# Onr/Council-GAN

Hardware: NVIDIA H100
Metric: training images/sec (gen+dis step) (higher is better)
Workload: dtype tf32

## Files before the change

council_gan_b200/csrc/api.cu:

```cuda
#include "common.cuh"
#include <string.h>

namespace cg {

static thread_local char g_err[512] = "";
std::atomic<uint64_t> g_launches{0};
thread_local int g_tc_mode = 7;
thread_local int g_pdl = 0;

void set_error(const char* fmt, ...) {
    va_list ap;
    va_start(ap, fmt);
    vsnprintf(g_err, sizeof(g_err), fmt, ap);
    va_end(ap);
}

int validate_geom(const cg_conv_geom& g) {
    CG_REQUIRE(g.G >= 1 && (g.x_groups == 1 || g.x_groups == g.G), "conv: x_groups=%d must be 1 or G=%d", g.x_groups, g.G);
    CG_REQUIRE(g.Cin % 4 == 0 && g.Cin > 0, "conv: Cin=%d must be a positive multiple of 4", g.Cin);
    CG_REQUIRE(g.Cout > 0 && g.B > 0 && g.H > 0 && g.W > 0, "conv: empty tensor");
    CG_REQUIRE(g.stride >= 1 && g.KH >= 1 && g.KW >= 1 && g.pad >= 0, "conv: bad kernel geometry");
    int Hin = g.ups ? 2 * g.H : g.H, Win = g.ups ? 2 * g.W : g.W;
    int Ho = (Hin + 2 * g.pad - g.KH) / g.stride + 1, Wo = (Win + 2 * g.pad - g.KW) / g.stride + 1;
    CG_REQUIRE(Ho == g.Ho && Wo == g.Wo, "conv: output size %dx%d inconsistent with geometry (expected %dx%d)", g.Ho, g.Wo, Ho, Wo);
// ... 83 lines not shown
        set_error("cudaGetDevice: %s", cudaGetErrorString(e));
        return CG_ERR_NO_DEVICE;
    }
    cudaDeviceProp prop;
    e = cudaGetDeviceProperties(&prop, dev);
    if (e != cudaSuccess) {
        set_error("cudaGetDeviceProperties: %s", cudaGetErrorString(e));
        return CG_ERR_NO_DEVICE;
    }
    if (sm_count) *sm_count = prop.multiProcessorCount;
    if (cc_major) *cc_major = prop.major;
    if (cc_minor) *cc_minor = prop.minor;
    return prop.multiProcessorCount;
}

extern "C" int cg_set_tensor_core_mode(int mode) {
    int prev = g_tc_mode;
    g_tc_mode = mode == 1 ? 7 : (mode & 7);
    g_small_bn = ((mode >> 23) & 1) ? 0 : 1;
    g_wgrad_tma = ((mode >> 25) & 1) ? 0 : 1;
    g_pdl = (mode >> 22) & 1;
    g_tc_serial_epilogue = (mode >> 26) & 1;
    g_tc_reg_epilogue = (mode >> 27) & 1;
    return prev;
}

extern "C" uint64_t cg_launch_count(void) { return g_launches.load(); }
extern "C" void cg_tensor_map_cache_stats(uint64_t* hits, uint64_t* misses) { tc_map_cache_stats(hits, misses); }

extern "C" int cg_zero(void* ptr, size_t bytes, void* stream) {
    cudaError_t e = cudaMemsetAsync(ptr, 0, bytes, (cudaStream_t)stream);
    if (e != cudaSuccess) {
        set_error("cg_zero: %s", cudaGetErrorString(e));
        return CG_ERR_CUDA;
    }
    return CG_OK;
}

extern "C" size_t cg_conv_workspace_bytes(const cg_conv_geom* g, int which) {
    if (!g) return 0;
    ConvDims d = conv_dims(*g);
    size_t need = 0;
    const bool patch_fwd = which == 0 && (g_tc_mode & 1) && patch_path(*g) && g->KH * g->KW >= 16;
    if (which == 2 && small_wgrad_supported(*g)) return small_ws(*g, 2);
    if (which == 1 && small_dgrad_supported(*g)) return small_ws(*g, 1);
    const bool patch_wgrad = which == 2 && (g_tc_mode & 4) && patch_path(*g);
// ... 138 lines not shown
```

council_gan_b200/csrc/common.cuh:

```cuda
#pragma once
#include <cuda.h>
#include <cuda_runtime.h>
#include <stdint.h>
#include <stdio.h>
#include <stdarg.h>
#include <atomic>
#include "../../include/council_b200.h"

namespace cg {

void set_error(const char* fmt, ...);
extern std::atomic<uint64_t> g_launches;
extern thread_local int g_tc_mode;
extern thread_local int g_small_bn;
extern thread_local int g_wgrad_tma;
extern thread_local int g_tc_serial_epilogue;
extern thread_local int g_tc_reg_epilogue;

constexpr int CG_MAX_DEVICES = 64;
inline int current_device() {
    int dev = 0;
    cudaGetDevice(&dev);
    return dev >= 0 && dev < CG_MAX_DEVICES ? dev : 0;
}
struct PerDeviceOnce {
    std::atomic<bool> done[CG_MAX_DEVICES];
    bool first() { return !done[current_device()].exchange(true); }
    void reset() { done[current_device()].store(false); }
};

inline int check_launch(const char* what) {
    g_launches.fetch_add(1, std::memory_order_relaxed);
    cudaError_t e = cudaGetLastError();
    if (e != cudaSuccess) {
        set_error("%s: %s", what, cudaGetErrorString(e));
        return CG_ERR_CUDA;
    }
    return CG_OK;
}

// ... 93 lines not shown
```

council_gan_b200/csrc/conv_tc.cu:

```cuda
#include "common.cuh"
#include "tc_ptx.cuh"
#include <cstdlib>
#include <cstdio>
#include <cuda.h>
#include <mutex>
#include <string.h>

namespace cg {

typedef CUresult (*EncodeTiledFn)(CUtensorMap*, CUtensorMapDataType, cuuint32_t, void*, const cuuint64_t*, const cuuint64_t*,
                                  const cuuint32_t*, const cuuint32_t*, CUtensorMapInterleave, CUtensorMapSwizzle,
                                  CUtensorMapL2promotion, CUtensorMapFloatOOBfill);
typedef CUresult (*EncodeIm2colFn)(CUtensorMap*, CUtensorMapDataType, cuuint32_t, void*, const cuuint64_t*, const cuuint64_t*,
                                   const int*, const int*, cuuint32_t, cuuint32_t, const cuuint32_t*, CUtensorMapInterleave,
                                   CUtensorMapSwizzle, CUtensorMapL2promotion, CUtensorMapFloatOOBfill);
typedef CUresult (*ReplaceAddressFn)(CUtensorMap*, void*);
static EncodeTiledFn g_encode_tiled = nullptr;
static ReplaceAddressFn g_replace_address = nullptr;
static EncodeIm2colFn g_encode_im2col = nullptr;
static int g_sm_count_dev[CG_MAX_DEVICES] = {0};
static int sm_count_now() {
    int dev = current_device();
    if (!g_sm_count_dev[dev]) cudaDeviceGetAttribute(&g_sm_count_dev[dev], cudaDevAttrMultiProcessorCount, dev);
    return g_sm_count_dev[dev];
}
thread_local int g_small_bn = 1;
thread_local int g_tc_serial_epilogue = 0;
thread_local int g_tc_reg_epilogue = 0;
static int g_driver_version = 0;
static std::once_flag g_once;

struct MapKey {
    const void* ptr;
    int64_t a, b;
    int32_t v[8];
    bool operator==(const MapKey& o) const { return ptr == o.ptr && a == o.a && b == o.b && memcmp(v, o.v, sizeof(v)) == 0; }
};
struct MapSlot {
    MapKey key;
    CUtensorMap map;
    bool used;
};
constexpr int MAP_SLOTS = 8192;
static MapSlot* g_map_cache = nullptr;
static std::mutex g_map_mutex;
static std::atomic<uint64_t> g_map_hits{0}, g_map_misses{0};
static inline uint32_t map_hash(const MapKey& k) {
    uint64_t h = 1469598103934665603ull;
    const unsigned char* p = reinterpret_cast<const unsigned char*>(&k);
    for (size_t i = 0; i < sizeof(MapKey); i++) h = (h ^ p[i]) * 1099511628211ull;
    return (uint32_t)(h ^ (h >> 32)) & (MAP_SLOTS - 1);
// ... 57 lines not shown
struct TcParams {
    CUtensorMap bmap;
    TcClass cls[TC_MAX_CLASSES];
    int ncls;
    int G, xg_images;
    int B, P, Q;
    int Cin, Cout, KH, KW, stride;
    int bn;
    int bk;
    int cps;
    int n_store;
    int out_H, out_W, out_sh, out_sw;
    int w_rows_per_group;
    float* y; const float* bias; const float* addend; const float* mask_src;
    float* stats;
    long stats_gbc;
    int act; float slope;
    int stages;
    int serial_epilogue;
    CUtensorMap ymap, addmap, maskmap;
    int epi_slots, epi_slot_bytes;
};

__device__ __forceinline__ void tc_tile(const TcParams& p, int t, int MT, int NT, int& mt, int& nt, int& c, int& g) {
    if (p.serial_epilogue) {
        mt = t % MT;
        int r = t / MT;
        nt = r % NT;
        r /= NT;
        c = r % p.ncls;
        g = r / p.ncls;
        return;
    }
    c = t % p.ncls;
    int r = t / p.ncls;
    mt = r % MT;
    r /= MT;
    nt = r % NT;
    g = r / NT;
}

__device__ __forceinline__ void tc_half_coords(const TcParams& p, int g, int mt, int h, int& q, int& n) {
    const int pq = p.P * p.Q;
    const int m = mt * TC_BM + 64 * h;
    const int img = m / pq, rem = m - img * pq;
    const int pp = rem / p.Q;
    q = rem - pp * p.Q;
    n = (g * p.B + img) * (p.out_H / p.out_sh) + pp;
}

template <int BK, int BN>
__global__ void __launch_bounds__(TC_THREADS, 1) conv_tc_kernel(const __grid_constant__ TcParams p) {
    pdl_trigger();
    extern __shared__ __align__(1024) uint8_t smem_raw[];
    uint8_t* smem = reinterpret_cast<uint8_t*>((reinterpret_cast<uintptr_t>(smem_raw) + 1023) & ~(uintptr_t)1023);
    const int wg = __shfl_sync(0xffffffffu, threadIdx.x >> 7, 0), tid = threadIdx.x & 127;
    constexpr int a_bytes = TC_BM * BK * 4;
    constexpr int b_bytes = ((BN * BK * 4) + 1023) & ~1023;
    const int stage_bytes = p.cps * (a_bytes + b_bytes);
    constexpr int tx_chunk = a_bytes + BN * BK * 4;
    constexpr bool tma_epi = BK == 32 && BN >= 64;
    const int epi_slots = tma_epi ? p.epi_slots : 0;
    uint8_t* epi = smem + (size_t)p.stages * stage_bytes;
    uint64_t* full_bar = reinterpret_cast<uint64_t*>(epi + (size_t)epi_slots * p.epi_slot_bytes);
    uint64_t* empty_bar = full_bar + p.stages;
    uint64_t* efull_bar = empty_bar + p.stages;
    uint64_t* eempty_bar = efull_bar + epi_slots;

    const int MT = (p.B * p.P * p.Q + TC_BM - 1) / TC_BM;
    const int NT = (p.Cout + BN - 1) / BN;
    const int tiles = p.G * p.ncls * NT * MT;
    const int kchunks = (p.Cin + BK - 1) / BK;
    const int kiters = p.KH * p.KW * kchunks;

    if (threadIdx.x == 0) {
        prefetch_tmap(&p.bmap);
        for (int c = 0; c < p.ncls; c++) prefetch_tmap(&p.cls[c].amap);
        for (int s = 0; s < p.stages; s++) {
            mbar_init(&full_bar[s], 1);
            mbar_init(&empty_bar[s], 2);
        }
        if (epi_slots) {
            prefetch_tmap(&p.ymap);
            if (p.addend) prefetch_tmap(&p.addmap);
            if (p.mask_src) prefetch_tmap(&p.maskmap);
        }
        for (int s = 0; s < epi_slots; s++) {
            mbar_init(&efull_bar[s], 1);
            mbar_init(&eempty_bar[s], 2);
        }
        fence_barrier_init();
    }
    __syncthreads();
    pdl_wait();

    if (wg == 0) {
        if (tid == 0) {
            int stage = 0;
            uint32_t phase = 0;
            for (int t = blockIdx.x; t < tiles; t += gridDim.x) {
                int mt, nt, c, g;
                tc_tile(p, t, MT, NT, mt, nt, c, g);
                const TcClass& cl = p.cls[c];
                long m0 = (long)mt * TC_BM;
                int img = (int)(m0 / (p.P * p.Q));
                int rem = (int)(m0 - (long)img * p.P * p.Q);
                int pp = rem / p.Q, qq = rem - pp * p.Q;
                int n_coord = g * p.xg_images + img;
                int w_coord = cl.w0 + qq * p.stride;
                int h_coord = cl.h0 + pp * p.stride;
                int wrow = g * p.w_rows_per_group + cl.wrow_off + nt * BN;
                int kh = 0, kw = 0, kc = 0;
                for (int k0 = 0; k0 < kiters; k0 += p.cps) {
                    const int n = kiters - k0 < p.cps ? kiters - k0 : p.cps;
                    mbar_wait(&empty_bar[stage], phase ^ 1);
                    uint8_t* sa = smem + (size_t)stage * stage_bytes;
                    uint8_t* sb = sa + p.cps * a_bytes;
                    mbar_expect_tx(&full_bar[stage], (uint32_t)(n * tx_chunk));
                    for (int j = 0; j < n; j++) {
                        tma_load_im2col_4d(&cl.amap, &full_bar[stage], sa + j * a_bytes, kc * BK, w_coord, h_coord, n_coord, (uint16_t)kw,
                                           (uint16_t)kh);
                        tma_load_2d(&p.bmap, &full_bar[stage], sb + j * b_bytes, (kh * p.KW + kw) * p.Cin + kc * BK, wrow);
                        if (++kc == kchunks) { kc = 0; if (++kw == p.KW) { kw = 0; ++kh; } }
                    }
                    if (++stage == p.stages) { stage = 0; phase ^= 1; }
                }
            }
        } else if (tid == 32 && epi_slots) {
            const uint32_t ebytes = (p.addend ? 2 * 8192 : 0) + (p.mask_src ? 2 * 8192 : 0);
            int es = 0;
            uint32_t ephase = 0;
            for (int t = blockIdx.x; t < tiles; t += gridDim.x) {
                int mt, nt, c, g;
                tc_tile(p, t, MT, NT, mt, nt, c, g);
                const TcClass& cl = p.cls[c];
                int q[2], n[2];
                tc_half_coords(p, g, mt, 0, q[0], n[0]);
                tc_half_coords(p, g, mt, 1, q[1], n[1]);
                for (int sl = 0; sl < BN / 32; sl++) {
                    mbar_wait(&eempty_bar[es], ephase ^ 1);
                    if (ebytes) {
                        mbar_expect_tx(&efull_bar[es], ebytes);
                        uint8_t* dst = epi + (size_t)es * p.epi_slot_bytes;
                        const int c0 = nt * BN + 32 * sl;
                        for (int h = 0; h < 2; h++) {
                            if (p.addend) tma_load_5d(&p.addmap, &efull_bar[es], dst + h * 8192, c0, cl.out_w0, q[h], cl.out_h0, n[h]);
                            if (p.mask_src)
                                tma_load_5d(&p.maskmap, &efull_bar[es], dst + (p.addend ? 16384 : 0) + h * 8192, c0, cl.out_w0, q[h],
                                            cl.out_h0, n[h]);
                        }
                    } else {
                        mbar_arrive(&efull_bar[es]);
                    }
                    if (++es == epi_slots) { es = 0; ephase ^= 1; }
                }
            }
        }
        return;
    }

    const int cw = wg - 1;
    const int warp4 = tid >> 5, lane = tid & 31;
    const int row0 = cw * 64 + warp4 * 16 + (lane >> 2);
    const int cq = 2 * (lane & 3);
    const uint64_t desc0 = BK == 32 ? make_kmajor_sw128_desc(0) : make_kmajor_sw32_desc(0);
    float acc[BN / 2];
    int stage = 0;
    uint32_t phase = 0;
    int es = 0;
    uint32_t ephase = 0;
    for (int t = blockIdx.x; t < tiles; t += gridDim.x) {
        int mt, nt, c, g;
        tc_tile(p, t, MT, NT, mt, nt, c, g);
        const TcClass& cl = p.cls[c];
        int prev = -1;
        for (int k0 = 0; k0 < kiters; k0 += p.cps) {
            const int n = kiters - k0 < p.cps ? kiters - k0 : p.cps;
            mbar_wait(&full_bar[stage], phase);
            const uint32_t sa = smem_u32(smem + (size_t)stage * stage_bytes) + cw * (64 * BK * 4);
            const uint32_t sb = smem_u32(smem + (size_t)stage * stage_bytes) + p.cps * a_bytes;
            wgmma_fence();
            for (int j = 0; j < n; j++) {
                const uint64_t adesc = desc0 | (uint64_t)(((sa + j * a_bytes) & 0x3FFFF) >> 4);
                const uint64_t bdesc = desc0 | (uint64_t)(((sb + j * b_bytes) & 0x3FFFF) >> 4);
#pragma unroll
                for (int kk = 0; kk < BK / 8; kk++)
                    wgmma_tf32<BN>(acc, adesc + (uint64_t)(kk * 2), bdesc + (uint64_t)(kk * 2), (k0 | j | kk) != 0 ? 1 : 0);
            }
            wgmma_commit();
            wgmma_wait<1>();
            if (prev >= 0 && tid == 0) mbar_arrive(&empty_bar[prev]);
            prev = stage;
            if (++stage == p.stages) { stage = 0; phase ^= 1; }
        }
        wgmma_wait<0>();
        wgmma_reg_fence(acc, BN / 2);
        if (tid == 0) mbar_arrive(&empty_bar[prev]);

        const int pq = p.P * p.Q;
        long out_off[2];
        bool valid[2];
#pragma unroll
        for (int h = 0; h < 2; h++) {
            const int m = mt * TC_BM + row0 + 8 * h;
            valid[h] = m < p.B * pq;
            out_off[h] = 0;
            if (valid[h]) {
                int img = m / pq;
                int rem = m - img * pq;
                int pp = rem / p.Q, qq = rem - pp * p.Q;
                long pix = ((long)(g * p.B + img) * p.out_H + (pp * p.out_sh + cl.out_h0)) * p.out_W + (qq * p.out_sw + cl.out_w0);
                out_off[h] = pix * p.Cout + nt * p.n_store;
            }
        }
        if (p.stats) {
            const int tiles_per_img = pq / TC_BM;
            const int img = (mt * TC_BM) / pq;
            const int chunk = ((c * tiles_per_img + (mt - img * tiles_per_img)) << 3) + cw * 4 + warp4;
            const bool b2 = lane & 4, b3 = lane & 8;
            float* st = p.stats + ((long)chunk * p.stats_gbc + (long)(g * p.B + img) * p.Cout + nt * BN + cq) * 2 + (b3 ? 2 : 0) + (b2 ? 1 : 0);
#pragma unroll
            for (int j = 0; j < BN / 8; j++) {
                const float s0 = acc[4 * j] + acc[4 * j + 2], s1 = acc[4 * j + 1] + acc[4 * j + 3];
                const float q0 = acc[4 * j] * acc[4 * j] + acc[4 * j + 2] * acc[4 * j + 2];
                const float q1 = acc[4 * j + 1] * acc[4 * j + 1] + acc[4 * j + 3] * acc[4 * j + 3];
                const float k0 = b2 ? q0 : s0, k1 = b2 ? q1 : s1;
                const float r0 = __shfl_xor_sync(0xffffffffu, b2 ? s0 : q0, 4), r1 = __shfl_xor_sync(0xffffffffu, b2 ? s1 : q1, 4);
                const float x0 = k0 + r0, x1 = k1 + r1;
                float v = (b3 ? x1 : x0) + __shfl_xor_sync(0xffffffffu, b3 ? x0 : x1, 8);
                v += __shfl_xor_sync(0xffffffffu, v, 16);
                if (lane < 16) st[16 * j] = v;
            }
        }
        if constexpr (tma_epi) {
            if (epi_slots) {
                int q, n;
                tc_half_coords(p, g, mt, cw, q, n);
                const int r0 = warp4 * 16 + (lane >> 2);
#pragma unroll
                for (int sl = 0; sl < BN / 32; sl++) {
                    float2 bv[4];
#pragma unroll
                    for (int jj = 0; jj < 4; jj++)
                        bv[jj] = p.bias ? __ldg(reinterpret_cast<const float2*>(p.bias + (long)g * p.Cout + nt * BN + 32 * sl + 8 * jj + cq))
                                        : make_float2(0.f, 0.f);
                    mbar_wait(&efull_bar[es], ephase);
                    uint8_t* half = epi + (size_t)es * p.epi_slot_bytes + cw * 8192;
                    const uint8_t* msk = half + (p.addend ? 16384 : 0);
#pragma unroll
                    for (int jj = 0; jj < 4; jj++) {
                        const int j = 4 * sl + jj;
#pragma unroll
                        for (int h = 0; h < 2; h++) {
                            const int r = r0 + 8 * h;
                            const int off = r * 128 + (((2 * jj + (cq >> 2)) ^ (r & 7)) << 4) + (cq & 3) * 4;
                            float2 o = make_float2(acc[4 * j + 2 * h] + bv[jj].x, acc[4 * j + 2 * h + 1] + bv[jj].y);
                            if (p.addend) {
                                const float2 a = *reinterpret_cast<const float2*>(half + off);
                                o.x += a.x; o.y += a.y;
                            }
                            if (p.mask_src) {
                                const float2 a = *reinterpret_cast<const float2*>(msk + off);
                                o.x *= a.x > 0.f ? 1.f : p.slope; o.y *= a.y > 0.f ? 1.f : p.slope;
                            } else if (p.act != CG_ACT_NONE) {
                                o.x = apply_act(o.x, p.act, p.slope); o.y = apply_act(o.y, p.act, p.slope);
                            }
                            *reinterpret_cast<float2*>(half + off) = o;
                        }
                    }
                    fence_proxy_async();
                    named_bar_sync(1 + cw, 128);
                    if (tid == 0) {
                        tma_store_5d(&p.ymap, half, nt * BN + 32 * sl, cl.out_w0, q, cl.out_h0, n);
                        bulk_commit();
                        if (sl > 0) {
                            bulk_wait_read<1>();
                            mbar_arrive(&eempty_bar[es == 0 ? epi_slots - 1 : es - 1]);
                        }
                        if (sl == BN / 32 - 1) {
                            bulk_wait_read<0>();
                            mbar_arrive(&eempty_bar[es]);
                        }
                    }
                    if (++es == epi_slots) { es = 0; ephase ^= 1; }
                }
                continue;
            }
        }
        if (!(p.addend || p.mask_src) || p.serial_epilogue) {
#pragma unroll
            for (int j = 0; j < BN / 8; j++) {
                const int col = 8 * j + cq;
// ... 52 lines not shown


static int encode_weights_map_raw(CUtensorMap* map, const float* w, long rows, long ktot, int bn, int bk) {
    cuuint64_t dims[2] = {(cuuint64_t)ktot, (cuuint64_t)rows};
    cuuint64_t strides[1] = {(cuuint64_t)ktot * 4};
    cuuint32_t box[2] = {(cuuint32_t)bk, (cuuint32_t)bn};
    cuuint32_t estr[2] = {1, 1};
    CUresult r = g_encode_tiled(map, CU_TENSOR_MAP_DATA_TYPE_TFLOAT32, 2, (void*)w, dims, strides, box, estr,
                                CU_TENSOR_MAP_INTERLEAVE_NONE, bk == 32 ? CU_TENSOR_MAP_SWIZZLE_128B : CU_TENSOR_MAP_SWIZZLE_32B,
                                CU_TENSOR_MAP_L2_PROMOTION_L2_256B, CU_TENSOR_MAP_FLOAT_OOB_FILL_NONE);
    if (r != CUDA_SUCCESS) {
        set_error("cuTensorMapEncodeTiled(weights rows=%ld ktot=%ld bn=%d) failed: %d", rows, ktot, bn, (int)r);
        return CG_ERR_CUDA;
    }
    return CG_OK;
}

static int encode_weights_map(CUtensorMap* map, const float* w, long rows, long ktot, int bn, int bk = TC_BK) {
    MapKey k{};
    k.ptr = w; k.a = rows; k.b = ktot; k.v[0] = bn; k.v[1] = bk; k.v[7] = 1;
    return cached_map(map, k, [&](CUtensorMap* m) { return encode_weights_map_raw(m, w, rows, ktot, bn, bk); });
}

static int encode_weights_map_p(TcParams& p, const float* w, long rows, long ktot) {
    return encode_weights_map(&p.bmap, w, rows, ktot, p.bn, p.bk);
}

static int encode_act_map_raw(CUtensorMap* map, const float* x, long N, int H, int W, int C, int lo_w, int lo_h, int up_w, int up_h,
                              int stride, int bk) {
    cuuint64_t dims[4] = {(cuuint64_t)C, (cuuint64_t)W, (cuuint64_t)H, (cuuint64_t)N};
    cuuint64_t strides[3] = {(cuuint64_t)C * 4, (cuuint64_t)W * C * 4, (cuuint64_t)H * W * C * 4};
    int lower[2] = {lo_w, lo_h};
    int upper[2] = {up_w, up_h};
    cuuint32_t estr[4] = {1, (cuuint32_t)stride, (cuuint32_t)stride, 1};
    CUresult r = g_encode_im2col(map, CU_TENSOR_MAP_DATA_TYPE_TFLOAT32, 4, (void*)x, dims, strides, lower, upper, bk, TC_BM, estr,
                                 CU_TENSOR_MAP_INTERLEAVE_NONE, bk == 32 ? CU_TENSOR_MAP_SWIZZLE_128B : CU_TENSOR_MAP_SWIZZLE_32B,
                                 CU_TENSOR_MAP_L2_PROMOTION_L2_128B, CU_TENSOR_MAP_FLOAT_OOB_FILL_NONE);
    if (r != CUDA_SUCCESS) {
        set_error("cuTensorMapEncodeIm2col(N=%ld H=%d W=%d C=%d corners %d,%d / %d,%d stride %d) failed: %d", N, H, W, C, lo_w, lo_h,
                  up_w, up_h, stride, (int)r);
        return CG_ERR_CUDA;
    }
    if (g_driver_version <= 13010 && (long)N * H * W * C * 4 < 131072) reinterpret_cast<uint64_t*>(map)[1] &= ~(1ull << 21);
    return CG_OK;
}

static int encode_act_map(CUtensorMap* map, const float* x, long N, int H, int W, int C, int lo_w, int lo_h, int up_w, int up_h,
                          int stride, int bk = TC_BK) {
    MapKey k{};
    k.ptr = x; k.a = N; k.b = ((int64_t)H << 32) | (uint32_t)W;
// ... 49 lines not shown

bool tc_fwd_supported(const cg_conv_geom& g) {
    init_driver();
    if (!g_encode_tiled || !g_encode_im2col) return false;
    if (g.ups && !(g.KH == 3 && g.KW == 3 && g.stride == 1 && g.pad == 1 && g.Cin % TC_BK == 0)) return false;
    if (pick_bk(g.Cin) == 0) return false;
    if (pick_bn(g.Cout) == 0) return false;
    if (g.pad > 120 || g.KH > 120) return false;
    if ((long)g.B * (g.ups ? g.H * g.W : g.Ho * g.Wo) < TC_BM) return false;
    return true;
}

template <int BK>
static void (*tc_kernel_for(int bn))(TcParams) {
    switch (bn) {
        case 16: return conv_tc_kernel<BK, 16>;
        case 64: return conv_tc_kernel<BK, 64>;
        case 128: return conv_tc_kernel<BK, 128>;
        case 256: return conv_tc_kernel<BK, 256>;
    }
    return nullptr;
}

static int launch_tc(TcParams& p, cudaStream_t st) {
    int a_bytes = TC_BM * p.bk * 4, b_bytes = ((p.bn * p.bk * 4) + 1023) & ~1023;
    int chunk_bytes = a_bytes + b_bytes;
    int kiters = p.KH * p.KW * ((p.Cin + p.bk - 1) / p.bk);
    int cps = p.bn <= 64 ? 2 : 1;
    if (p.bk == 8) cps = 8;
    while (cps > 1 && (cps > kiters || cps * chunk_bytes > 64 * 1024)) cps >>= 1;
    p.cps = cps;
    int stage_bytes = cps * chunk_bytes;
    int stages = (226 * 1024 - 1024 - 2 * TC_MAX_STAGES * 8) / stage_bytes;
    if (stages > TC_MAX_STAGES) stages = TC_MAX_STAGES;
    if (stages > 4 && stage_bytes >= 48 * 1024) stages = 4;
    if (p.n_store == 0) p.n_store = p.bn;
    p.serial_epilogue = g_tc_serial_epilogue;
    p.epi_slots = 0;
    const int nops = (p.addend ? 1 : 0) + (p.mask_src ? 1 : 0);
    const bool aligned = ((uintptr_t)p.y | (uintptr_t)p.addend | (uintptr_t)p.mask_src) % 16 == 0;
    if (g_replace_address && !g_tc_reg_epilogue && !p.serial_epilogue && p.bk == TC_BK && p.bn >= 64 && p.n_store == p.bn && (long)p.P * p.Q % TC_BM == 0 &&
        (p.Q % 64 == 0 || 64 % p.Q == 0) && p.out_H % p.out_sh == 0 && p.out_W % p.out_sw == 0 && p.Cout % 4 == 0 && aligned) {
        const int slot_bytes = (nops ? nops : 1) * 16384;
        auto slots_beside = [&](int st) { return (int)((227L * 1024 - 1024 - (long)st * stage_bytes - 2 * st * 8) / (slot_bytes + 16)); };
        while (slots_beside(stages) < 2 && stages > 4) stages--;
        const int e = slots_beside(stages);
        if (e >= 2) {
            p.epi_slots = e < 4 ? e : 4;
            p.epi_slot_bytes = slot_bytes;
            const long ni = (long)p.G * p.B;
            const int qbox = p.Q < 64 ? p.Q : 64;
            if (int rc = encode_out_map(&p.ymap, p.y, ni, p.out_H, p.out_W, p.Cout, p.out_sh, p.out_sw, qbox)) return rc;
            if (p.addend)
                if (int rc = encode_out_map(&p.addmap, p.addend, ni, p.out_H, p.out_W, p.Cout, p.out_sh, p.out_sw, qbox)) return rc;
            if (p.mask_src)
                if (int rc = encode_out_map(&p.maskmap, p.mask_src, ni, p.out_H, p.out_W, p.Cout, p.out_sh, p.out_sw, qbox)) return rc;
        }
    }
    p.stages = stages;
    size_t smem = (size_t)stages * stage_bytes + 1024  + 2 * stages * 8 + (size_t)p.epi_slots * (p.epi_slot_bytes + 16);
    void (*kern)(TcParams) = p.bk == 32 ? tc_kernel_for<32>(p.bn) : tc_kernel_for<8>(p.bn);
    if (!kern) {
        set_error("conv_tc: no kernel for N tile %d / K chunk %d", p.bn, p.bk);
        return CG_ERR_ARG;
    }
    static PerDeviceOnce attr_set;
    if (attr_set.first()) {
        for (int bn : {16, 64, 128, 256}) {
            cudaError_t e = cudaFuncSetAttribute(tc_kernel_for<32>(bn), cudaFuncAttributeMaxDynamicSharedMemorySize, 227 * 1024);
            if (e == cudaSuccess) e = cudaFuncSetAttribute(tc_kernel_for<8>(bn), cudaFuncAttributeMaxDynamicSharedMemorySize, 227 * 1024);
            if (e != cudaSuccess) {
                attr_set.reset();
                set_error("cudaFuncSetAttribute(conv_tc_kernel): %s", cudaGetErrorString(e));
                return CG_ERR_CUDA;
            }
        }
    }
    int MT = cdiv((long)p.B * p.P * p.Q, TC_BM);
    long tiles = (long)p.G * p.ncls * ((p.Cout + p.bn - 1) / p.bn) * MT;
    const long slots = sm_count_now();
    int grid = (int)(tiles < slots ? tiles : slots);
    launch_k(kern, grid, TC_THREADS, smem, st, p);
    return check_launch("conv_tc_kernel");
}


__global__ void ups_weight_transform_kernel(const float* __restrict__ w, float* __restrict__ wc, long total, int Cout, int Cin) {
    pdl_trigger();
    pdl_wait();
    long i = (long)blockIdx.x * blockDim.x + threadIdx.x;
    if (i >= total) return;
    int ci = (int)(i % Cin);
    long t = i / Cin;
    int ss = (int)(t % 2); t /= 2;
    int r = (int)(t % 2); t /= 2;
    int co = (int)(t % Cout); t /= Cout;
    int cls = (int)(t % 4);
    int g = (int)(t / 4);
// ... 22 lines not shown
                size_t ws_bytes, cudaStream_t st, float* stats_part) {
    init_driver();
    TcParams p{};
    p.stats = stats_part;
    p.stats_gbc = (long)g.G * g.B * g.Cout;
    p.bn = pick_bn(g.Cout);
    if (p.bn > 64) p.bn = fill_bn(p.bn, (long)g.B * (g.ups ? g.H * g.W : g.Ho * g.Wo), g.G * (g.ups ? 4 : 1), g.Cout);
    p.n_store = p.bn == 16 ? g.Cout : p.bn;
    p.bk = pick_bk(g.Cin);
    long nimg = (long)(g.x_groups == 1 ? 1 : g.G) * g.B;
    p.G = g.G; p.xg_images = g.x_groups == 1 ? 0 : g.B;
    p.B = g.B; p.Cin = g.Cin; p.Cout = g.Cout;
    p.y = y; p.bias = bias; p.addend = nullptr; p.mask_src = nullptr; p.act = act; p.slope = slope;
    if (g.ups) {
        size_t need = tc_fwd_ws(g);
        if (need > ws_bytes) {
            set_error("conv_fwd(tc, upsample classes): workspace %zu < %zu bytes", ws_bytes, need);
            return CG_ERR_WORKSPACE;
        }
        float* wc = (float*)ws;
        long total = (long)g.G * 4 * g.Cout * 4 * g.Cin;
        launch_k(ups_weight_transform_kernel, cdiv(total, 256), 256, 0, st, w, wc, total, g.Cout, g.Cin);
        if (int rc = check_launch("ups_weight_transform")) return rc;
        if (int rc = encode_weights_map_p(p, wc, (long)g.G * 4 * g.Cout, 4L * g.Cin)) return rc;
        for (int c = 0; c < 4; c++) {
            int a = c >> 1, b = c & 1;
            int lo_h = a == 0 ? -1 : 0, lo_w = b == 0 ? -1 : 0;
            int up_h = a == 0 ? -1 : 0, up_w = b == 0 ? -1 : 0;
            if (int rc = encode_act_map(&p.cls[c].amap, x, nimg, g.H, g.W, g.Cin, lo_w, lo_h, up_w, up_h, 1, p.bk)) return rc;
            p.cls[c].w0 = lo_w; p.cls[c].h0 = lo_h; p.cls[c].out_h0 = a; p.cls[c].out_w0 = b; p.cls[c].wrow_off = c * g.Cout;
        }
        p.ncls = 4;
        p.P = g.H; p.Q = g.W; p.KH = 2; p.KW = 2; p.stride = 1;
        p.out_H = g.Ho; p.out_W = g.Wo; p.out_sh = 2; p.out_sw = 2;
        p.w_rows_per_group = 4 * g.Cout;
        return launch_tc(p, st);
    }
    long ktot = (long)g.KH * g.KW * g.Cin;
    if (int rc = encode_weights_map_p(p, w, (long)g.G * g.Cout, ktot)) return rc;
    if (int rc = encode_act_map(&p.cls[0].amap, x, nimg, g.H, g.W, g.Cin, -g.pad, -g.pad, g.pad - (g.KW - 1), g.pad - (g.KH - 1), g.stride,
                                p.bk))
        return rc;
    p.cls[0].w0 = -g.pad; p.cls[0].h0 = -g.pad; p.cls[0].out_h0 = 0; p.cls[0].out_w0 = 0; p.cls[0].wrow_off = 0;
    p.ncls = 1;
    p.P = g.Ho; p.Q = g.Wo;
    p.KH = g.KH; p.KW = g.KW; p.stride = g.stride;
    p.out_H = g.Ho; p.out_W = g.Wo; p.out_sh = 1; p.out_sw = 1;
    p.w_rows_per_group = g.Cout;
    return launch_tc(p, st);
}

__global__ void __launch_bounds__(256) dgrad_weight_transform_kernel(const float* __restrict__ w, float* __restrict__ wt, int Cout, int Cin,
                                                                     int CinP, int KH, int KW, int s) {
    pdl_trigger();
    pdl_wait();
    __shared__ float tile[32][33];
    const int TH = KH / s, TW = KW / s;
    const int cit = (CinP + 31) / 32;
    const int co0 = (blockIdx.x / cit) * 32, ci0 = (blockIdx.x % cit) * 32;
    int t = blockIdx.y;
    const int ss = t % TW; t /= TW;
    const int r = t % TH; t /= TH;
    const int cls = t;
    const int g = blockIdx.z;
    const int ph = cls / s, pw = cls - ph * s;
    const int kh = ph + s * (TH - 1 - r), kw = pw + s * (TW - 1 - ss);
    const int tx = threadIdx.x, ty = threadIdx.y;
#pragma unroll
    for (int j = 0; j < 4; j++) {
        const int co = co0 + ty + 8 * j, ci = ci0 + tx;
        tile[ty + 8 * j][tx] = (co < Cout && ci < Cin) ? __ldg(w + ((((long)g * Cout + co) * KH + kh) * KW + kw) * Cin + ci) : 0.f;
    }
// ... 30 lines not shown
    init_driver();
    size_t need = tc_dgrad_ws(g);
    if (need > ws_bytes) {
        set_error("conv_dgrad(tc): workspace %zu < %zu bytes", ws_bytes, need);
        return CG_ERR_WORKSPACE;
    }
    const int s = g.stride, TH = g.KH / s, TW = g.KW / s, ncls = s * s;
    const int Hin = g.ups ? 2 * g.H : g.H, Win = g.ups ? 2 * g.W : g.W;
    float* wt = (float*)ws;
    const int CinP = g.Cin <= 16 ? 16 : g.Cin;
    size_t wt_bytes = ((size_t)g.G * g.Cout * g.KH * g.KW * CinP * sizeof(float) + 1023) & ~(size_t)1023;
    float* d_seen = g.ups ? (float*)((uint8_t*)ws + wt_bytes) : dx;
    long total = (long)g.G * g.Cout * g.KH * g.KW * CinP;
    (void)total;
    launch_k(dgrad_weight_transform_kernel, dim3(cdiv(g.Cout, 32) * cdiv(CinP, 32), g.KH * g.KW, g.G), dim3(32, 8), 0, st, w, wt, g.Cout, g.Cin, CinP,
                                                                                                                  g.KH, g.KW, s);
    if (int rc = check_launch("dgrad_weight_transform")) return rc;

    TcParams p{};
    p.bn = pick_bn(g.Cin);
    if (p.bn > 64) p.bn = fill_bn(p.bn, (long)g.B * ((g.ups ? 2 * g.H : g.H) / g.stride) * ((g.ups ? 2 * g.W : g.W) / g.stride), g.G * g.stride * g.stride, g.Cin);
    p.n_store = p.bn == 16 ? g.Cin : p.bn;
    p.bk = pick_bk(g.Cout);
    long ktot = (long)TH * TW * g.Cout;
    if (int rc = encode_weights_map_p(p, wt, (long)g.G * ncls * CinP, ktot)) return rc;
    for (int c = 0; c < ncls; c++) {
        int ph = c / s, pw = c - ph * s;
        int ihf = ((ph - g.pad) % s + s) % s, iwf = ((pw - g.pad) % s + s) % s;
        int padl_h = (TH - 1) - (ihf + g.pad - ph) / s, padl_w = (TW - 1) - (iwf + g.pad - pw) / s;
        int Hc = Hin / s, Wc = Win / s;
        int up_h = Hc - g.Ho - padl_h, up_w = Wc - g.Wo - padl_w;
        if (int rc = encode_act_map(&p.cls[c].amap, dy, (long)g.G * g.B, g.Ho, g.Wo, g.Cout, -padl_w, -padl_h, up_w, up_h, 1, p.bk)) return rc;
        p.cls[c].w0 = -padl_w; p.cls[c].h0 = -padl_h;
        p.cls[c].out_h0 = ihf; p.cls[c].out_w0 = iwf;
        p.cls[c].wrow_off = c * CinP;
    }
    p.ncls = ncls;
    p.G = g.G; p.xg_images = g.B;
    p.B = g.B; p.P = Hin / s; p.Q = Win / s;
    p.Cin = g.Cout; p.Cout = g.Cin; p.KH = TH; p.KW = TW; p.stride = 1;
    p.out_H = Hin; p.out_W = Win; p.out_sh = s; p.out_sw = s;
    p.w_rows_per_group = ncls * CinP;
    p.y = d_seen; p.bias = nullptr;
    p.addend = g.ups ? nullptr : addend; p.mask_src = g.ups ? nullptr : mask_src;
    p.act = CG_ACT_NONE; p.slope = mask_slope;
    if (int rc = launch_tc(p, st)) return rc;
    if (g.ups) return pool2x2_sum(d_seen, dx, addend, mask_src, mask_slope, (long)g.G * g.B, g.H, g.W, g.Cin, st);
    return CG_OK;
}


constexpr int WG_BK = 32;

struct WgParams {
    const float* x; const float* dy; float* out;
    int G, xg_images, B, H, W, Ho, Wo, Cin, Cout, KH, KW, stride, pad;
    long Mpix, chunk;
    int ci_tiles;
};

__device__ __forceinline__ float f4_at(const float4& v, int j) { return j == 0 ? v.x : j == 1 ? v.y : j == 2 ? v.z : v.w; }

__device__ __forceinline__ void store_kmajor4(uint8_t* tile, int r0, int k, const float4& v) {
#pragma unroll
    for (int j = 0; j < 4; j++) {
        const int r = r0 + j;
        *reinterpret_cast<float*>(tile + (r >> 3) * 1024 + (r & 7) * 128 + (((k >> 2) ^ (r & 7)) << 4) + (k & 3) * 4) = to_tf32(f4_at(v, j));
    }
}
// ... 517 lines not shown
```

council_gan_b200/csrc/tc_ptx.cuh:

```cuda
#pragma once
#include <cuda.h>
#include <cuda_runtime.h>
#include <stdint.h>

namespace cg {

__device__ __forceinline__ uint32_t smem_u32(const void* p) { return (uint32_t)__cvta_generic_to_shared(p); }

__device__ __forceinline__ void mbar_init(uint64_t* bar, uint32_t count) {
    asm volatile("mbarrier.init.shared::cta.b64 [%0], %1;" ::"r"(smem_u32(bar)), "r"(count));
}
__device__ __forceinline__ void mbar_expect_tx(uint64_t* bar, uint32_t bytes) {
    asm volatile("mbarrier.arrive.expect_tx.shared::cta.b64 _, [%0], %1;" ::"r"(smem_u32(bar)), "r"(bytes) : "memory");
}
__device__ __forceinline__ void mbar_arrive(uint64_t* bar) {
    asm volatile("mbarrier.arrive.shared::cta.b64 _, [%0];" ::"r"(smem_u32(bar)) : "memory");
}
__device__ __forceinline__ void mbar_wait(uint64_t* bar, uint32_t parity) {
    uint32_t done;
    const uint32_t addr = smem_u32(bar);
    do {
        asm volatile(
            "{\n"
            ".reg .pred p;\n"
// ... 25 lines not shown
__device__ __forceinline__ void tma_load_4d(const CUtensorMap* map, uint64_t* bar, void* dst, int c0, int c1, int c2, int c3) {
    asm volatile(
        "cp.async.bulk.tensor.4d.shared::cluster.global.mbarrier::complete_tx::bytes [%0], [%1, {%3, %4, %5, %6}], [%2];" ::"r"(smem_u32(dst)),
        "l"(map), "r"(smem_u32(bar)), "r"(c0), "r"(c1), "r"(c2), "r"(c3)
        : "memory");
}
__device__ __forceinline__ void tma_load_5d(const CUtensorMap* map, uint64_t* bar, void* dst, int c0, int c1, int c2, int c3, int c4) {
    asm volatile(
        "cp.async.bulk.tensor.5d.shared::cluster.global.mbarrier::complete_tx::bytes [%0], [%1, {%3, %4, %5, %6, %7}], [%2];" ::"r"(smem_u32(dst)),
        "l"(map), "r"(smem_u32(bar)), "r"(c0), "r"(c1), "r"(c2), "r"(c3), "r"(c4)
        : "memory");
}
__device__ __forceinline__ void tma_store_5d(const CUtensorMap* map, const void* src, int c0, int c1, int c2, int c3, int c4) {
    asm volatile("cp.async.bulk.tensor.5d.global.shared::cta.tile.bulk_group [%0, {%2, %3, %4, %5, %6}], [%1];" ::"l"(map),
                 "r"(smem_u32(src)), "r"(c0), "r"(c1), "r"(c2), "r"(c3), "r"(c4)
                 : "memory");
}
__device__ __forceinline__ void bulk_commit() { asm volatile("cp.async.bulk.commit_group;" ::: "memory"); }
template <int N>
__device__ __forceinline__ void bulk_wait_read() { asm volatile("cp.async.bulk.wait_group.read %0;" ::"n"(N) : "memory"); }
template <int N>
__device__ __forceinline__ void bulk_wait() { asm volatile("cp.async.bulk.wait_group %0;" ::"n"(N) : "memory"); }
__device__ __forceinline__ void named_bar_sync(int id, int count) { asm volatile("bar.sync %0, %1;" ::"r"(id), "r"(count) : "memory"); }
__device__ __forceinline__ void prefetch_tmap(const CUtensorMap* map) {
    asm volatile("prefetch.tensormap [%0];" ::"l"(map) : "memory");
}

__device__ __forceinline__ uint64_t make_kmajor_sw128_desc(uint32_t smem_addr) {
    uint64_t d = 0;
    d |= (uint64_t)((smem_addr & 0x3FFFF) >> 4);
    d |= (uint64_t)1 << 16;
    d |= (uint64_t)(1024 >> 4) << 32;
    d |= (uint64_t)1 << 62;
    return d;
}
__device__ __forceinline__ uint64_t make_kmajor_sw32_desc(uint32_t smem_addr) {
    uint64_t d = 0;
    d |= (uint64_t)((smem_addr & 0x3FFFF) >> 4);
    d |= (uint64_t)1 << 16;
    d |= (uint64_t)(256 >> 4) << 32;
    d |= (uint64_t)3 << 62;
    return d;
}

__device__ __forceinline__ void wgmma_fence() { asm volatile("wgmma.fence.sync.aligned;" ::: "memory"); }
__device__ __forceinline__ void wgmma_commit() { asm volatile("wgmma.commit_group.sync.aligned;" ::: "memory"); }
// ... 78 lines not shown
```

Baseline: 46.74.

## Add ping-pong consumer warpgroup schedule for short-K tensor-core convolutions

Adds a ping-pong variant of the TMA/wgmma convolution kernel. The two consumer warpgroups each own whole 128x128 tiles and alternate, coordinating through named barriers, so one group's epilogue (stats, bias/activation, TMA store) overlaps the other's MMA mainloop. It also reallocates registers with setmaxnreg. It is selected for short-K convs with enough tiles and forces the N tile to 128. The change adds barrier complexity and ring-skip bookkeeping and can be disabled by a new cooperative mode bit.

```diff
diff --git a/council_gan_b200/csrc/api.cu b/council_gan_b200/csrc/api.cu
--- a/council_gan_b200/csrc/api.cu
+++ b/council_gan_b200/csrc/api.cu
@@ -129,6 +129,7 @@
     g_pdl = (mode >> 22) & 1;
     g_tc_serial_epilogue = (mode >> 26) & 1;
     g_tc_reg_epilogue = (mode >> 27) & 1;
+    g_tc_cooperative = (mode >> 28) & 1;
     return prev;
 }
 
diff --git a/council_gan_b200/csrc/common.cuh b/council_gan_b200/csrc/common.cuh
--- a/council_gan_b200/csrc/common.cuh
+++ b/council_gan_b200/csrc/common.cuh
@@ -16,6 +16,7 @@
 extern thread_local int g_wgrad_tma;
 extern thread_local int g_tc_serial_epilogue;
 extern thread_local int g_tc_reg_epilogue;
+extern thread_local int g_tc_cooperative;
 
 constexpr int CG_MAX_DEVICES = 64;
 inline int current_device() {
diff --git a/council_gan_b200/csrc/conv_tc.cu b/council_gan_b200/csrc/conv_tc.cu
--- a/council_gan_b200/csrc/conv_tc.cu
+++ b/council_gan_b200/csrc/conv_tc.cu
@@ -27,6 +27,7 @@
 thread_local int g_small_bn = 1;
 thread_local int g_tc_serial_epilogue = 0;
 thread_local int g_tc_reg_epilogue = 0;
+thread_local int g_tc_cooperative = 0;
 static int g_driver_version = 0;
 static std::once_flag g_once;
 
@@ -130,7 +131,17 @@
     int epi_slots, epi_slot_bytes;
 };
 
+template <bool PP>
 __device__ __forceinline__ void tc_tile(const TcParams& p, int t, int MT, int NT, int& mt, int& nt, int& c, int& g) {
+    if (PP) {
+        c = t % p.ncls;
+        int r = t / p.ncls;
+        nt = r % NT;
+        r /= NT;
+        mt = r % MT;
+        g = r / MT;
+        return;
+    }
     if (p.serial_epilogue) {
         mt = t % MT;
         int r = t / MT;
@@ -157,7 +168,69 @@
     n = (g * p.B + img) * (p.out_H / p.out_sh) + pp;
 }
 
-template <int BK, int BN>
+template <int BN>
+__device__ __forceinline__ void tc_stats(const TcParams& p, const float* acc, int c, int mt, int g, int nt, int mb, int warp4, int lane) {
+    const int pq = p.P * p.Q;
+    const int cq = 2 * (lane & 3);
+    const int tiles_per_img = pq / TC_BM;
+    const int img = (mt * TC_BM) / pq;
+    const int chunk = ((c * tiles_per_img + (mt - img * tiles_per_img)) << 3) + mb * 4 + warp4;
+    const bool b2 = lane & 4, b3 = lane & 8;
+    float* st = p.stats + ((long)chunk * p.stats_gbc + (long)(g * p.B + img) * p.Cout + nt * BN + cq) * 2 + (b3 ? 2 : 0) + (b2 ? 1 : 0);
+#pragma unroll
+    for (int j = 0; j < BN / 8; j++) {
+        const float s0 = acc[4 * j] + acc[4 * j + 2], s1 = acc[4 * j + 1] + acc[4 * j + 3];
+        const float q0 = acc[4 * j] * acc[4 * j] + acc[4 * j + 2] * acc[4 * j + 2];
+        const float q1 = acc[4 * j + 1] * acc[4 * j + 1] + acc[4 * j + 3] * acc[4 * j + 3];
+        const float k0 = b2 ? q0 : s0, k1 = b2 ? q1 : s1;
+        const float r0 = __shfl_xor_sync(0xffffffffu, b2 ? s0 : q0, 4), r1 = __shfl_xor_sync(0xffffffffu, b2 ? s1 : q1, 4);
+        const float x0 = k0 + r0, x1 = k1 + r1;
+        float v = (b3 ? x1 : x0) + __shfl_xor_sync(0xffffffffu, b3 ? x0 : x1, 8);
+        v += __shfl_xor_sync(0xffffffffu, v, 16);
+        if (lane < 16) st[16 * j] = v;
+    }
+}
+
+__device__ __forceinline__ void tc_epi_half(const TcParams& p, const float* acc, int sl, const float2* bv, uint8_t* half, int r0, int cq) {
+    const uint8_t* msk = half + (p.addend ? 16384 : 0);
+#pragma unroll
+    for (int jj = 0; jj < 4; jj++) {
+        const int j = 4 * sl + jj;
+#pragma unroll
+        for (int h = 0; h < 2; h++) {
+            const int r = r0 + 8 * h;
+            const int off = r * 128 + (((2 * jj + (cq >> 2)) ^ (r & 7)) << 4) + (cq & 3) * 4;
+            float2 o = make_float2(acc[4 * j + 2 * h] + bv[jj].x, acc[4 * j + 2 * h + 1] + bv[jj].y);
+            if (p.addend) {
+                const float2 a = *reinterpret_cast<const float2*>(half + off);
+                o.x += a.x; o.y += a.y;
+            }
+            if (p.mask_src) {
+                const float2 a = *reinterpret_cast<const float2*>(msk + off);
+                o.x *= a.x > 0.f ? 1.f : p.slope; o.y *= a.y > 0.f ? 1.f : p.slope;
+            } else if (p.act != CG_ACT_NONE) {
+                o.x = apply_act(o.x, p.act, p.slope); o.y = apply_act(o.y, p.act, p.slope);
+            }
+            *reinterpret_cast<float2*>(half + off) = o;
+        }
+    }
+}
+
+template <int BN>
+__device__ __forceinline__ void tc_slice_bias(const TcParams& p, int g, int nt, int sl, int cq, float2* bv) {
+#pragma unroll
+    for (int jj = 0; jj < 4; jj++)
+        bv[jj] = p.bias ? __ldg(reinterpret_cast<const float2*>(p.bias + (long)g * p.Cout + nt * BN + 32 * sl + 8 * jj + cq))
+                        : make_float2(0.f, 0.f);
+}
+
+__device__ __forceinline__ void ring_skip(int& slot, uint32_t& phase, int n, int slots) {
+    slot += n;
+    phase ^= (uint32_t)(slot / slots) & 1;
+    slot %= slots;
+}
+
+template <int BK, int BN, bool PP = false>
 __global__ void __launch_bounds__(TC_THREADS, 1) conv_tc_kernel(const __grid_constant__ TcParams p) {
     pdl_trigger();
     extern __shared__ __align__(1024) uint8_t smem_raw[];
@@ -186,7 +259,7 @@
         for (int c = 0; c < p.ncls; c++) prefetch_tmap(&p.cls[c].amap);
         for (int s = 0; s < p.stages; s++) {
             mbar_init(&full_bar[s], 1);
-            mbar_init(&empty_bar[s], 2);
+            mbar_init(&empty_bar[s], PP ? 1 : 2);
         }
         if (epi_slots) {
             prefetch_tmap(&p.ymap);
@@ -195,20 +268,24 @@
         }
         for (int s = 0; s < epi_slots; s++) {
             mbar_init(&efull_bar[s], 1);
-            mbar_init(&eempty_bar[s], 2);
+            mbar_init(&eempty_bar[s], PP ? 1 : 2);
         }
         fence_barrier_init();
     }
     __syncthreads();
     pdl_wait();
 
+    if constexpr (PP) {
+        if (wg == 0) setmaxnreg_dec<40>();
+        else setmaxnreg_inc<232>();
+    }
     if (wg == 0) {
         if (tid == 0) {
             int stage = 0;
             uint32_t phase = 0;
             for (int t = blockIdx.x; t < tiles; t += gridDim.x) {
                 int mt, nt, c, g;
-                tc_tile(p, t, MT, NT, mt, nt, c, g);
+                tc_tile<PP>(p, t, MT, NT, mt, nt, c, g);
                 const TcClass& cl = p.cls[c];
                 long m0 = (long)mt * TC_BM;
                 int img = (int)(m0 / (p.P * p.Q));
@@ -240,7 +317,7 @@
             uint32_t ephase = 0;
             for (int t = blockIdx.x; t < tiles; t += gridDim.x) {
                 int mt, nt, c, g;
-                tc_tile(p, t, MT, NT, mt, nt, c, g);
+                tc_tile<PP>(p, t, MT, NT, mt, nt, c, g);
                 const TcClass& cl = p.cls[c];
                 int q[2], n[2];
                 tc_half_coords(p, g, mt, 0, q[0], n[0]);
@@ -269,17 +346,99 @@
 
     const int cw = wg - 1;
     const int warp4 = tid >> 5, lane = tid & 31;
-    const int row0 = cw * 64 + warp4 * 16 + (lane >> 2);
     const int cq = 2 * (lane & 3);
     const uint64_t desc0 = BK == 32 ? make_kmajor_sw128_desc(0) : make_kmajor_sw32_desc(0);
-    float acc[BN / 2];
     int stage = 0;
     uint32_t phase = 0;
     int es = 0;
     uint32_t ephase = 0;
+    if constexpr (PP) {
+        static_assert(BK == 32 && BN >= 64, "the ping-pong schedule runs the shared-memory epilogue only");
+        const int r0 = warp4 * 16 + (lane >> 2);
+        const int kstages = (kiters + p.cps - 1) / p.cps;
+        float acc[2][BN / 2];
+        if (cw) {
+            ring_skip(stage, phase, kstages, p.stages);
+            ring_skip(es, ephase, BN / 32, epi_slots);
+        }
+        for (int i = cw, t = blockIdx.x + cw * gridDim.x; t < tiles; i += 2, t += 2 * gridDim.x) {
+            int mt, nt, c, g;
+            tc_tile<PP>(p, t, MT, NT, mt, nt, c, g);
+            const TcClass& cl = p.cls[c];
+            if (i > 0) named_bar_sync(3 + cw, 256);
+            int prev = -1;
+            for (int k0 = 0; k0 < kiters; k0 += p.cps) {
+                const int n = kiters - k0 < p.cps ? kiters - k0 : p.cps;
+                mbar_wait(&full_bar[stage], phase);
+                const uint32_t sa = smem_u32(smem + (size_t)stage * stage_bytes);
+                const uint32_t sb = sa + p.cps * a_bytes;
+                wgmma_fence();
+                for (int j = 0; j < n; j++) {
+                    const uint64_t adesc = desc0 | (uint64_t)(((sa + j * a_bytes) & 0x3FFFF) >> 4);
+                    const uint64_t bdesc = desc0 | (uint64_t)(((sb + j * b_bytes) & 0x3FFFF) >> 4);
+#pragma unroll
+                    for (int kk = 0; kk < BK / 8; kk++) {
+                        wgmma_tf32<BN>(acc[0], adesc + (uint64_t)(kk * 2), bdesc + (uint64_t)(kk * 2), (k0 | j | kk) != 0 ? 1 : 0);
+                        wgmma_tf32<BN>(acc[1], adesc + (uint64_t)((64 * BK * 4) >> 4) + (uint64_t)(kk * 2), bdesc + (uint64_t)(kk * 2),
+                                       (k0 | j | kk) != 0 ? 1 : 0);
+                    }
+                }
+                wgmma_commit();
+                wgmma_wait<1>();
+                if (prev >= 0 && tid == 0) mbar_arrive(&empty_bar[prev]);
+                prev = stage;
+                if (++stage == p.stages) { stage = 0; phase ^= 1; }
+            }
+            if (t + gridDim.x < tiles) named_bar_arrive(3 + (cw ^ 1), 256);
+            wgmma_wait<0>();
+            wgmma_reg_fence(acc[0], BN / 2);
+            wgmma_reg_fence(acc[1], BN / 2);
+            if (tid == 0) mbar_arrive(&empty_bar[prev]);
+            if (p.stats) {
+                tc_stats<BN>(p, acc[0], c, mt, g, nt, 0, warp4, lane);
+                tc_stats<BN>(p, acc[1], c, mt, g, nt, 1, warp4, lane);
+            }
+            int q[2], n[2];
+            tc_half_coords(p, g, mt, 0, q[0], n[0]);
+            tc_half_coords(p, g, mt, 1, q[1], n[1]);
+            if (i > 0) named_bar_sync(5 + cw, 256);
+#pragma unroll
+            for (int sl = 0; sl < BN / 32; sl++) {
+                float2 bv[4];
+                tc_slice_bias<BN>(p, g, nt, sl, cq, bv);
+                mbar_wait(&efull_bar[es], ephase);
+                uint8_t* slot = epi + (size_t)es * p.epi_slot_bytes;
+                tc_epi_half(p, acc[0], sl, bv, slot, r0, cq);
+                tc_epi_half(p, acc[1], sl, bv, slot + 8192, r0, cq);
+                fence_proxy_async();
+                named_bar_sync(1 + cw, 128);
+                if (tid == 0) {
+                    tma_store_5d(&p.ymap, slot, nt * BN + 32 * sl, cl.out_w0, q[0], cl.out_h0, n[0]);
+                    tma_store_5d(&p.ymap, slot + 8192, nt * BN + 32 * sl, cl.out_w0, q[1], cl.out_h0, n[1]);
+                    bulk_commit();
+                    if (sl > 0) {
+                        bulk_wait_read<1>();
+                        mbar_arrive(&eempty_bar[es == 0 ? epi_slots - 1 : es - 1]);
+                    }
+                    if (sl == BN / 32 - 1) {
+                        bulk_wait_read<0>();
+                        mbar_arrive(&eempty_bar[es]);
+                    }
+                }
+                if (++es == epi_slots) { es = 0; ephase ^= 1; }
+            }
+            if (t + gridDim.x < tiles) named_bar_arrive(5 + (cw ^ 1), 256);
+            ring_skip(stage, phase, kstages, p.stages);
+            ring_skip(es, ephase, BN / 32, epi_slots);
+        }
+        if (tid == 0) bulk_wait<0>();
+        return;
+    }
+    const int row0 = cw * 64 + warp4 * 16 + (lane >> 2);
+    float acc[BN / 2];
     for (int t = blockIdx.x; t < tiles; t += gridDim.x) {
         int mt, nt, c, g;
-        tc_tile(p, t, MT, NT, mt, nt, c, g);
+        tc_tile<PP>(p, t, MT, NT, mt, nt, c, g);
         const TcClass& cl = p.cls[c];
         int prev = -1;
         for (int k0 = 0; k0 < kiters; k0 += p.cps) {
@@ -321,25 +480,7 @@
                 out_off[h] = pix * p.Cout + nt * p.n_store;
             }
         }
-        if (p.stats) {
-            const int tiles_per_img = pq / TC_BM;
-            const int img = (mt * TC_BM) / pq;
-            const int chunk = ((c * tiles_per_img + (mt - img * tiles_per_img)) << 3) + cw * 4 + warp4;
-            const bool b2 = lane & 4, b3 = lane & 8;
-            float* st = p.stats + ((long)chunk * p.stats_gbc + (long)(g * p.B + img) * p.Cout + nt * BN + cq) * 2 + (b3 ? 2 : 0) + (b2 ? 1 : 0);
-#pragma unroll
-            for (int j = 0; j < BN / 8; j++) {
-                const float s0 = acc[4 * j] + acc[4 * j + 2], s1 = acc[4 * j + 1] + acc[4 * j + 3];
-                const float q0 = acc[4 * j] * acc[4 * j] + acc[4 * j + 2] * acc[4 * j + 2];
-                const float q1 = acc[4 * j + 1] * acc[4 * j + 1] + acc[4 * j + 3] * acc[4 * j + 3];
-                const float k0 = b2 ? q0 : s0, k1 = b2 ? q1 : s1;
-                const float r0 = __shfl_xor_sync(0xffffffffu, b2 ? s0 : q0, 4), r1 = __shfl_xor_sync(0xffffffffu, b2 ? s1 : q1, 4);
-                const float x0 = k0 + r0, x1 = k1 + r1;
-                float v = (b3 ? x1 : x0) + __shfl_xor_sync(0xffffffffu, b3 ? x0 : x1, 8);
-                v += __shfl_xor_sync(0xffffffffu, v, 16);
-                if (lane < 16) st[16 * j] = v;
-            }
-        }
+        if (p.stats) tc_stats<BN>(p, acc, c, mt, g, nt, cw, warp4, lane);
         if constexpr (tma_epi) {
             if (epi_slots) {
                 int q, n;
@@ -348,34 +489,10 @@
 #pragma unroll
                 for (int sl = 0; sl < BN / 32; sl++) {
                     float2 bv[4];
-#pragma unroll
-                    for (int jj = 0; jj < 4; jj++)
-                        bv[jj] = p.bias ? __ldg(reinterpret_cast<const float2*>(p.bias + (long)g * p.Cout + nt * BN + 32 * sl + 8 * jj + cq))
-                                        : make_float2(0.f, 0.f);
+                    tc_slice_bias<BN>(p, g, nt, sl, cq, bv);
                     mbar_wait(&efull_bar[es], ephase);
                     uint8_t* half = epi + (size_t)es * p.epi_slot_bytes + cw * 8192;
-                    const uint8_t* msk = half + (p.addend ? 16384 : 0);
-#pragma unroll
-                    for (int jj = 0; jj < 4; jj++) {
-                        const int j = 4 * sl + jj;
-#pragma unroll
-                        for (int h = 0; h < 2; h++) {
-                            const int r = r0 + 8 * h;
-                            const int off = r * 128 + (((2 * jj + (cq >> 2)) ^ (r & 7)) << 4) + (cq & 3) * 4;
-                            float2 o = make_float2(acc[4 * j + 2 * h] + bv[jj].x, acc[4 * j + 2 * h + 1] + bv[jj].y);
-                            if (p.addend) {
-                                const float2 a = *reinterpret_cast<const float2*>(half + off);
-                                o.x += a.x; o.y += a.y;
-                            }
-                            if (p.mask_src) {
-                                const float2 a = *reinterpret_cast<const float2*>(msk + off);
-                                o.x *= a.x > 0.f ? 1.f : p.slope; o.y *= a.y > 0.f ? 1.f : p.slope;
-                            } else if (p.act != CG_ACT_NONE) {
-                                o.x = apply_act(o.x, p.act, p.slope); o.y = apply_act(o.y, p.act, p.slope);
-                            }
-                            *reinterpret_cast<float2*>(half + off) = o;
-                        }
-                    }
+                    tc_epi_half(p, acc, sl, bv, half, r0, cq);
                     fence_proxy_async();
                     named_bar_sync(1 + cw, 128);
                     if (tid == 0) {
@@ -474,10 +591,6 @@
     return cached_map(map, k, [&](CUtensorMap* m) { return encode_weights_map_raw(m, w, rows, ktot, bn, bk); });
 }
 
-static int encode_weights_map_p(TcParams& p, const float* w, long rows, long ktot) {
-    return encode_weights_map(&p.bmap, w, rows, ktot, p.bn, p.bk);
-}
-
 static int encode_act_map_raw(CUtensorMap* map, const float* x, long N, int H, int W, int C, int lo_w, int lo_h, int up_w, int up_h,
                               int stride, int bk) {
     cuuint64_t dims[4] = {(cuuint64_t)C, (cuuint64_t)W, (cuuint64_t)H, (cuuint64_t)N};
@@ -573,7 +686,26 @@
     return nullptr;
 }
 
-static int launch_tc(TcParams& p, cudaStream_t st) {
+constexpr int TC_PP_SHORT_K = 36;
+constexpr int TC_PP_STATS_K = 72;
+static bool use_pingpong(const TcParams& p, bool tma_geom) {
+    if (g_tc_cooperative || !tma_geom || p.bk != TC_BK || (p.bn != 128 && p.bn != 256)) return false;
+    const int kchunks = p.KH * p.KW * ((p.Cin + p.bk - 1) / p.bk);
+    const long tiles = (long)p.G * p.ncls * (p.Cout / 128) * cdiv((long)p.B * p.P * p.Q, TC_BM);
+    if (tiles < 2L * sm_count_now()) return false;
+    return kchunks <= TC_PP_SHORT_K || (p.stats && p.bn == 256 && kchunks <= TC_PP_STATS_K);
+}
+
+static int launch_tc(TcParams& p, const float* w, long wrows, long wktot, cudaStream_t st) {
+    if (p.n_store == 0) p.n_store = p.bn;
+    p.serial_epilogue = g_tc_serial_epilogue;
+    const bool aligned = ((uintptr_t)p.y | (uintptr_t)p.addend | (uintptr_t)p.mask_src) % 16 == 0;
+    const bool tma_geom = g_replace_address && !g_tc_reg_epilogue && !p.serial_epilogue && p.bk == TC_BK && p.bn >= 64 &&
+                          p.n_store == p.bn && (long)p.P * p.Q % TC_BM == 0 && (p.Q % 64 == 0 || 64 % p.Q == 0) &&
+                          p.out_H % p.out_sh == 0 && p.out_W % p.out_sw == 0 && p.Cout % 4 == 0 && aligned;
+    const bool pp = use_pingpong(p, tma_geom);
+    if (pp) p.bn = p.n_store = 128;
+    if (int rc = encode_weights_map(&p.bmap, w, wrows, wktot, p.bn, p.bk)) return rc;
     int a_bytes = TC_BM * p.bk * 4, b_bytes = ((p.bn * p.bk * 4) + 1023) & ~1023;
     int chunk_bytes = a_bytes + b_bytes;
     int kiters = p.KH * p.KW * ((p.Cin + p.bk - 1) / p.bk);
@@ -585,13 +717,9 @@
     int stages = (226 * 1024 - 1024 - 2 * TC_MAX_STAGES * 8) / stage_bytes;
     if (stages > TC_MAX_STAGES) stages = TC_MAX_STAGES;
     if (stages > 4 && stage_bytes >= 48 * 1024) stages = 4;
-    if (p.n_store == 0) p.n_store = p.bn;
-    p.serial_epilogue = g_tc_serial_epilogue;
     p.epi_slots = 0;
     const int nops = (p.addend ? 1 : 0) + (p.mask_src ? 1 : 0);
-    const bool aligned = ((uintptr_t)p.y | (uintptr_t)p.addend | (uintptr_t)p.mask_src) % 16 == 0;
-    if (g_replace_address && !g_tc_reg_epilogue && !p.serial_epilogue && p.bk == TC_BK && p.bn >= 64 && p.n_store == p.bn && (long)p.P * p.Q % TC_BM == 0 &&
-        (p.Q % 64 == 0 || 64 % p.Q == 0) && p.out_H % p.out_sh == 0 && p.out_W % p.out_sw == 0 && p.Cout % 4 == 0 && aligned) {
+    if (tma_geom) {
         const int slot_bytes = (nops ? nops : 1) * 16384;
         auto slots_beside = [&](int st) { return (int)((227L * 1024 - 1024 - (long)st * stage_bytes - 2 * st * 8) / (slot_bytes + 16)); };
         while (slots_beside(stages) < 2 && stages > 4) stages--;
@@ -611,6 +739,13 @@
     p.stages = stages;
     size_t smem = (size_t)stages * stage_bytes + 1024  + 2 * stages * 8 + (size_t)p.epi_slots * (p.epi_slot_bytes + 16);
     void (*kern)(TcParams) = p.bk == 32 ? tc_kernel_for<32>(p.bn) : tc_kernel_for<8>(p.bn);
+    if (pp) {
+        if (!p.epi_slots) {
+            set_error("conv_tc: ping-pong schedule without the shared-memory epilogue");
+            return CG_ERR_ARG;
+        }
+        kern = conv_tc_kernel<32, 128, true>;
+    }
     if (!kern) {
         set_error("conv_tc: no kernel for N tile %d / K chunk %d", p.bn, p.bk);
         return CG_ERR_ARG;
@@ -625,6 +760,12 @@
                 set_error("cudaFuncSetAttribute(conv_tc_kernel): %s", cudaGetErrorString(e));
                 return CG_ERR_CUDA;
             }
+        }
+        cudaError_t e = cudaFuncSetAttribute(conv_tc_kernel<32, 128, true>, cudaFuncAttributeMaxDynamicSharedMemorySize, 227 * 1024);
+        if (e != cudaSuccess) {
+            attr_set.reset();
+            set_error("cudaFuncSetAttribute(conv_tc_kernel, ping-pong): %s", cudaGetErrorString(e));
+            return CG_ERR_CUDA;
         }
     }
     int MT = cdiv((long)p.B * p.P * p.Q, TC_BM);
@@ -693,7 +834,6 @@
         long total = (long)g.G * 4 * g.Cout * 4 * g.Cin;
         launch_k(ups_weight_transform_kernel, cdiv(total, 256), 256, 0, st, w, wc, total, g.Cout, g.Cin);
         if (int rc = check_launch("ups_weight_transform")) return rc;
-        if (int rc = encode_weights_map_p(p, wc, (long)g.G * 4 * g.Cout, 4L * g.Cin)) return rc;
         for (int c = 0; c < 4; c++) {
             int a = c >> 1, b = c & 1;
             int lo_h = a == 0 ? -1 : 0, lo_w = b == 0 ? -1 : 0;
@@ -705,10 +845,8 @@
         p.P = g.H; p.Q = g.W; p.KH = 2; p.KW = 2; p.stride = 1;
         p.out_H = g.Ho; p.out_W = g.Wo; p.out_sh = 2; p.out_sw = 2;
         p.w_rows_per_group = 4 * g.Cout;
-        return launch_tc(p, st);
-    }
-    long ktot = (long)g.KH * g.KW * g.Cin;
-    if (int rc = encode_weights_map_p(p, w, (long)g.G * g.Cout, ktot)) return rc;
+        return launch_tc(p, wc, (long)g.G * 4 * g.Cout, 4L * g.Cin, st);
+    }
     if (int rc = encode_act_map(&p.cls[0].amap, x, nimg, g.H, g.W, g.Cin, -g.pad, -g.pad, g.pad - (g.KW - 1), g.pad - (g.KH - 1), g.stride,
                                 p.bk))
         return rc;
@@ -718,7 +856,7 @@
     p.KH = g.KH; p.KW = g.KW; p.stride = g.stride;
     p.out_H = g.Ho; p.out_W = g.Wo; p.out_sh = 1; p.out_sw = 1;
     p.w_rows_per_group = g.Cout;
-    return launch_tc(p, st);
+    return launch_tc(p, w, (long)g.G * g.Cout, (long)g.KH * g.KW * g.Cin, st);
 }
 
 __global__ void __launch_bounds__(256) dgrad_weight_transform_kernel(const float* __restrict__ w, float* __restrict__ wt, int Cout, int Cin,
@@ -795,8 +933,6 @@
     if (p.bn > 64) p.bn = fill_bn(p.bn, (long)g.B * ((g.ups ? 2 * g.H : g.H) / g.stride) * ((g.ups ? 2 * g.W : g.W) / g.stride), g.G * g.stride * g.stride, g.Cin);
     p.n_store = p.bn == 16 ? g.Cin : p.bn;
     p.bk = pick_bk(g.Cout);
-    long ktot = (long)TH * TW * g.Cout;
-    if (int rc = encode_weights_map_p(p, wt, (long)g.G * ncls * CinP, ktot)) return rc;
     for (int c = 0; c < ncls; c++) {
         int ph = c / s, pw = c - ph * s;
         int ihf = ((ph - g.pad) % s + s) % s, iwf = ((pw - g.pad) % s + s) % s;
@@ -817,7 +953,7 @@
     p.y = d_seen; p.bias = nullptr;
     p.addend = g.ups ? nullptr : addend; p.mask_src = g.ups ? nullptr : mask_src;
     p.act = CG_ACT_NONE; p.slope = mask_slope;
-    if (int rc = launch_tc(p, st)) return rc;
+    if (int rc = launch_tc(p, wt, (long)g.G * ncls * CinP, (long)TH * TW * g.Cout, st)) return rc;
     if (g.ups) return pool2x2_sum(d_seen, dx, addend, mask_src, mask_slope, (long)g.G * g.B, g.H, g.W, g.Cin, st);
     return CG_OK;
 }
diff --git a/council_gan_b200/csrc/tc_ptx.cuh b/council_gan_b200/csrc/tc_ptx.cuh
--- a/council_gan_b200/csrc/tc_ptx.cuh
+++ b/council_gan_b200/csrc/tc_ptx.cuh
@@ -71,6 +71,11 @@
 template <int N>
 __device__ __forceinline__ void bulk_wait() { asm volatile("cp.async.bulk.wait_group %0;" ::"n"(N) : "memory"); }
 __device__ __forceinline__ void named_bar_sync(int id, int count) { asm volatile("bar.sync %0, %1;" ::"r"(id), "r"(count) : "memory"); }
+__device__ __forceinline__ void named_bar_arrive(int id, int count) { asm volatile("bar.arrive %0, %1;" ::"r"(id), "r"(count) : "memory"); }
+template <int N>
+__device__ __forceinline__ void setmaxnreg_dec() { asm volatile("setmaxnreg.dec.sync.aligned.u32 %0;" ::"n"(N)); }
+template <int N>
+__device__ __forceinline__ void setmaxnreg_inc() { asm volatile("setmaxnreg.inc.sync.aligned.u32 %0;" ::"n"(N)); }
 __device__ __forceinline__ void prefetch_tmap(const CUtensorMap* map) {
     asm volatile("prefetch.tensormap [%0];" ::"l"(map) : "memory");
 }
```

Result: no change. 46.70, median of 6 (-0.1%).
